# AlphacatPlus/VmambaIR

Hardware: AMD Instinct MI355X
Metric: images/sec, x4 SR 64->256 training step (fwd+bwd+Adam+EMA), full VmambaIR UNet (higher is better)
Workload: dtype bf16; 1 GPU; BASELINE.json configs[1]: x4 SR 64x64 LQ, MambaSISR6 dim48 [15,1,1,1]+15, bf16 autocast (scan arithmetic f32), batch 8 per GPU; global_batch=8, per_gpu_batch=8, parallelism=dp1, step_launch=hipGraph replay, vendor_conv_solver_search=True, vendor_conv_solver_records=bench_data/miopen, optimizer=Adam 2e-4 (0.9,0.99) + EMA 0.999, loss=L1, rccl_ranks=1, allreduce_overlapped=False, allreduce_buckets=1, allreduce_bytes=0

## Files before the change

### include/vmambair_oss.h

```cpp
#ifndef VMAMBAIR_OSS_H
#define VMAMBAIR_OSS_H

#include <stddef.h>
#include <stdint.h>

#ifdef __cplusplus
extern "C" {
#endif

#define OSS_OK 0
#define OSS_ERR_NULL (-1)
#define OSS_ERR_SHAPE (-2)
#define OSS_ERR_DSTATE (-3)
#define OSS_ERR_WORKSPACE (-4)

#define OSS_MAX_DSTATE 256

typedef enum {
    OSS_F32 = 0, OSS_F16 = 1, OSS_BF16 = 2,
    OSS_F32_BF16X3 = 3
} oss_dtype;

typedef void *oss_stream_t;

// ... 101 lines not shown
                   float *dweight, float *dbias, float *partials, int batch, int hidden, int height, int width,
                   int64_t t_batch_stride, int64_t t_channel_stride, int64_t dout_batch_stride, int64_t dout_channel_stride,
                   int64_t dt_batch_stride, int64_t dt_channel_stride, oss_stream_t stream);

int oss_dwconv3x3_flat2_ok(oss_dtype io, int height, int width);
int oss_dwconv3x3_silu_flat2_fwd(oss_dtype io, const void *x, const float *weight, const float *bias, void *x2, int batch, int channels,
                                 int height, int width, int64_t x_batch_stride, int64_t x_channel_stride, oss_stream_t stream);
int oss_dwconv3x3_silu_flat2_bwd(oss_dtype io, const void *x, const float *weight, const float *bias, const void *g2, void *dx,
                                 float *dweight, float *dbias, float *partials, int batch, int channels, int height, int width,
                                 int64_t x_batch_stride, int64_t x_channel_stride, int64_t dx_batch_stride, int64_t dx_channel_stride,
                                 oss_stream_t stream);

int oss_conv1x1_fwd(oss_dtype io, const void *x, const float *weight, const float *bias, const void *residual, void *y,
                    int batch, int cout, int cin, int pixels, int64_t x_batch_stride, int64_t x_channel_stride,
                    oss_stream_t stream);
int oss_conv1x1_dgrad(oss_dtype io, const void *dy, const float *weight, void *dx, int batch, int cout, int cin, int pixels,
                      int64_t dy_batch_stride, int64_t dy_channel_stride, oss_stream_t stream);
size_t oss_conv1x1_wgrad_partial_floats(int batch, int cout, int cin, int pixels);
int oss_conv1x1_wg(oss_dtype io, const void *x, const float *weight, const float *bias, void *y, int batch, int cout, int cin,
                   int pixels, int64_t x_batch_stride, int64_t x_channel_stride, int transposed_weight, oss_stream_t stream);
int oss_ln_conv1x1_ok(oss_dtype io, int cout, int cin, int pixels);
int oss_ln_conv1x1_fwd(oss_dtype io, const void *x, const float *ln_weight, const float *ln_bias, float eps, void *n, float *mean,
                       float *rstd, const float *weight, const float *bias, void *y, int batch, int cout, int cin, int pixels,
                       int64_t x_batch_stride, int64_t x_channel_stride, oss_stream_t stream);
int oss_conv1x1_dgrad_ln_bwd_ok(oss_dtype io, int cout, int cin, int pixels, int batch);
size_t oss_conv1x1_dgrad_ln_bwd_partial_floats(int batch, int cin, int pixels);
int oss_conv1x1_dgrad_ln_bwd(oss_dtype io, const void *dy, const float *weight, const void *x, const float *ln_weight, int ln_has_bias,
                             const float *mean, const float *rstd, const void *skip_grad, void *dx, float *dln_weight, float *dln_bias,
                             float *partials, int batch, int cout, int cin, int pixels, int64_t dy_batch_stride,
                             int64_t dy_channel_stride, oss_stream_t stream);
void oss_conv1x1_set_wg(int on, int pixels);
void oss_conv1x1_wgrad_set_tile(int mode);
void oss_conv1x1_wgrad_set_span(int mult);
int oss_conv1x1_wgrad(oss_dtype io, const void *dy, const void *x, float *dweight, float *dbias, float *partials, int batch,
                      int cout, int cin, int pixels, int64_t dy_batch_stride, int64_t dy_channel_stride,
                      int64_t x_batch_stride, int64_t x_channel_stride, oss_stream_t stream);

int oss_cross_scan2(oss_dtype in_type, oss_dtype out_type, const void *x, void *x2, int batch, int D, int height, int width,
                    int64_t x_batch_stride, int64_t x_channel_stride, oss_stream_t stream);
int oss_cross_merge2(oss_dtype io, const void *g2, void *dx, int batch, int D, int height, int width, oss_stream_t stream);
int oss_proj_fwd(oss_dtype io, const void *x2, const float *x_proj_weight, const float *dt_projs_weight, void *xdbl, void *dts,
                 int batch, int D, int C, int R, int seqlen, oss_stream_t stream);
int oss_proj_dgrad(oss_dtype io, const void *ddts, void *dxdbl, const void *du, const float *x_proj_weight,
                   const float *dt_projs_weight, void *dx2, int batch, int D, int C, int R, int seqlen, oss_stream_t stream);
size_t oss_proj_wgrad_partial_floats(int batch, int D, int C, int R, int seqlen);
void oss_proj_set_path(int force_vector_alu);
int oss_proj_rows_optional_ok(oss_dtype io, int batch, int D, int C, int R, int seqlen);
int oss_proj_wgrad(oss_dtype io, const void *x2, const void *xdbl, const void *dxdbl, const void *ddts, float *dx_proj_weight,
                   float *ddt_projs_weight, float *partials, int batch, int D, int C, int R, int seqlen, oss_stream_t stream);

typedef struct {
    int B, L, dc, Rc, Cc, reserved_;
    const float *pooled;
    const float *cin_w, *cin_b;
    const float *Wxc;
    const float *Wdtc;
    const float *dt_bias;
    const float *A_logs;
    const float *Dsc;
    const float *cout_w, *cout_b;
    const float *cn_w, *cn_b;
    float *zt;
    float *dts;
    float *hs;
    float *y;
    float *yc;
// ... 131 lines not shown
```

### vmambair_amd/csrc/oss_capi.hip

```cpp
#include <atomic>
#include <cstdlib>
#include <mutex>
#include <vector>
#include <cstring>
#include <algorithm>
#include "oss_device.h"
#include "oss_host.h"

namespace oss {

static std::atomic<int> g_force_fwd{-1}, g_force_bwd{-1};
static std::atomic<int> g_last_fwd{-1}, g_last_bwd{-1};
static std::atomic<int> g_force_fwd_seg{-1}, g_force_bwd_seg{-1};
std::atomic<int> g_last_fwd_segments{1}, g_last_bwd_segments{1}, g_last_bwd_lane_states{0};

int scan_pick_segments(long wgs, int n_chunks, int seg_req, double ovh) {
    if (seg_req == 0 || seg_req == 1 || n_chunks < 2 || wgs <= 0) return 1;
    if (seg_req > 1) return std::min(std::min(seg_req, n_chunks), kMaxSegments);
    if (wgs >= 256) return 1;
    int best = 1;
    double best_cost = (double)n_chunks;
    for (int s = 2; s <= std::min(n_chunks, 16); ++s) {
        const int cps = (n_chunks + s - 1) / s;
        if ((n_chunks + cps - 1) / cps != s) continue;
// ... 487 lines not shown
int oss_ln_conv1x1_fwd(oss_dtype io, const void *x, const float *ln_weight, const float *ln_bias, float eps, void *n, float *mean,
                       float *rstd, const float *weight, const float *bias, void *y, int batch, int cout, int cin, int pixels,
                       int64_t xsb, int64_t xsc, oss_stream_t stream) {
    if (is_f32_split(io)) return OSS_ERR_SHAPE;
    fam_count(FAM_CONV1X1, (double)batch * pixels * (esz(io) * (2.0 * cin + cout) + 8.0) + 4.0 * cin * cout);
    if (!x || !ln_weight || !n || !mean || !rstd || !weight || !y) return OSS_ERR_NULL;
    if (batch <= 0 || batch > 65535) return OSS_ERR_SHAPE;
    return ln_conv1x1_wg(io, x, ln_weight, ln_bias, eps, n, mean, rstd, weight, bias, y, batch, cout, cin, pixels, xsb, xsc,
                         reinterpret_cast<hipStream_t>(stream));
}

int oss_conv1x1_dgrad_ln_bwd_ok(oss_dtype io, int cout, int cin, int pixels, int batch) {
    if (is_f32_split(io)) return 0;
    return conv1x1_dgrad_lnbwd_ok(io, cin, cout, pixels, batch);
}
size_t oss_conv1x1_dgrad_ln_bwd_partial_floats(int batch, int cin, int pixels) {
    if (batch <= 0 || cin <= 0 || pixels <= 0) return 0;
    return conv1x1_dgrad_lnbwd_partial_floats(batch, cin, pixels);
}
int oss_conv1x1_dgrad_ln_bwd(oss_dtype io, const void *dy, const float *weight, const void *x, const float *ln_weight, int ln_has_bias,
                             const float *mean, const float *rstd, const void *skip_grad, void *dx, float *dln_weight, float *dln_bias,
                             float *partials, int batch, int cout, int cin, int pixels, int64_t gsb, int64_t gsc, oss_stream_t stream) {
    if (is_f32_split(io)) return OSS_ERR_SHAPE;
    fam_count(FAM_CONV1X1, (double)batch * pixels * (esz(io) * ((double)cout + 2.0 * cin + (skip_grad ? cin : 0)) + 8.0) + 4.0 * cin * cout);
    if (!dy || !weight || !x || !ln_weight || !mean || !rstd || !dx || !dln_weight || !partials) return OSS_ERR_NULL;
    if (batch <= 0 || batch > 65535) return OSS_ERR_SHAPE;
    return conv1x1_dgrad_lnbwd(io, dy, weight, x, ln_weight, ln_has_bias, mean, rstd, skip_grad, dx, dln_weight, dln_bias, partials, batch,
                               cin, cout, pixels, gsb, gsc, reinterpret_cast<hipStream_t>(stream));
}

void oss_conv1x1_set_wg(int on, int pixels) { conv1x1_set_wg(on); conv1x1_wg_set_pixels(pixels); }
void oss_conv1x1_wgrad_set_tile(int mode) { conv1x1_wgrad_set_tile(mode); }
void oss_conv1x1_wgrad_set_span(int mult) { conv1x1_wgrad_set_span(mult); }

int oss_proj_wgrad(oss_dtype io, const void *x2, const void *xdbl, const void *dxdbl, const void *ddts, float *dx_proj_weight,
                   float *ddt_projs_weight, float *partials, int batch, int D, int C, int R, int seqlen, oss_stream_t stream) {
    const int x3 = take_f32_split(io);
    fam_count(FAM_WGRAD, (double)batch * seqlen * esz(io) * (2.0 * D + 8.0 * C + (ddts ? 4.0 * D : 0.0)));
    if (!x2 || !xdbl || !dxdbl || !dx_proj_weight || !partials) return OSS_ERR_NULL;
    if (ddts && !ddt_projs_weight) return OSS_ERR_NULL;
    if (batch <= 0 || D <= 0 || seqlen <= 0 || R <= 0 || C <= R) return OSS_ERR_SHAPE;
    hipStream_t s = reinterpret_cast<hipStream_t>(stream);
    const int64_t L = seqlen;
    if (io == OSS_F32) {
        int e = rows_f32_wgrad(reinterpret_cast<const float *>(dxdbl), reinterpret_cast<const float *>(x2), dx_proj_weight, partials, batch,
                               4, 2, C, D, seqlen, 4 * C * L, C * L, L, 2 * D * L, D * L, L, s, nullptr, x3);
        if (e || !ddts) return e;
        float *part2 = partials + (size_t)batch * conv1x1_wgrad_slabs(seqlen) * 2 * (2 * (size_t)C) * D;
        return rows_f32_wgrad(reinterpret_cast<const float *>(ddts), reinterpret_cast<const float *>(xdbl), ddt_projs_weight, part2, batch, 4,
                              4, D, R, seqlen, 4 * D * L, D * L, L, 4 * C * L, C * L, L, s, nullptr, x3);
    }
    int e = conv1x1_wgrad(io, dxdbl, x2, dx_proj_weight, partials, batch, 2 * C, D, seqlen, 4 * C * L, L, 2 * D * L, L, s,
                           2,  C * L,  D * L,  C,  2 * C * L);
    if (e || !ddts) return e;
    float *part2 = partials + (size_t)batch * conv1x1_wgrad_slabs(seqlen) * 2 * (2 * (size_t)C) * D;
    return conv1x1_wgrad(io, ddts, xdbl, ddt_projs_weight, part2, batch, D, R, seqlen, 4 * D * L, L, 4 * C * L, L, s,
                          4,  D * L,  C * L,  D, 0);
}

int oss_cross_scan2(oss_dtype in_type, oss_dtype out_type, const void *x, void *x2, int batch, int D, int height, int width,
                    int64_t x_batch_stride, int64_t x_channel_stride, oss_stream_t stream) {
    if (is_f32_split(in_type) || is_f32_split(out_type)) return OSS_ERR_SHAPE;
    fam_count(FAM_MERGE, (double)batch * D * height * width * (esz(in_type) + 2.0 * esz(out_type)));
    if (!x || !x2) return OSS_ERR_NULL;
    if (batch <= 0 || D <= 0 || height <= 0 || width <= 0) return OSS_ERR_SHAPE;
    return cross_scan2(in_type, out_type, x, x2, batch, D, height, width, x_batch_stride, x_channel_stride,
// ... 455 lines not shown
```

### vmambair_amd/csrc/oss_conv1x1.hip

```cpp
#include <atomic>
#include <cstdlib>
#include "oss_device.h"
#include "oss_global_ptr.h"
#include "oss_host.h"
#include "oss_mfma.h"

namespace oss {

template <typename T>
__global__ void __launch_bounds__(256)
oss_conv1x1_kernel(const T *__restrict__ x, const float *__restrict__ w, const float *__restrict__ bias, T *__restrict__ y,
                   int M, int K, int P, int64_t xsb, int64_t xsk, int64_t ws_m, int64_t ws_k, const T *__restrict__ res) {
    const int lane = threadIdx.x & 63, wave = threadIdx.x >> 6;
    const int b = blockIdx.y;
    const int m0 = blockIdx.z * 32;
    const int p0 = (blockIdx.x * 4 + wave) * 32;
    if (p0 >= P) return;
    const int col = lane & 31, kg = lane >> 5;
    const int p = p0 + col;
    const bool pok = p < P;
    const T *xb = x + b * xsb + (pok ? p : 0);
    T *yb = y + (size_t)b * M * P;
    const int mrow = m0 + col;
    const bool mok = mrow < M;
// ... 519 lines not shown
#pragma unroll
        for (int ks = 0; ks < KS; ++ks) {
#pragma unroll
            for (int e = 0; e < 8; ++e) {
                const int k = kc + ks * 16 + kg * 8 + e;
                const bool kok = k < K;
                const uint32_t raw = xw[(kok ? k : K - 1) * xsw];
                const uint32_t v = (pok && kok) ? raw : 0u;
                bfa[ks][e] = (short)(v & 0xffffu);
                bfb[ks][e] = (short)(v >> 16);
            }
        }
#pragma unroll
        for (int t = 0; t < MT; ++t) {
            s16x8 af[KS];
#pragma unroll
            for (int ks = 0; ks < KS; ++ks) af[ks] = load_wfrag<T, WT, WVEC>(w, (mt0 + t) * 32 + col, M, K, kc + ks * 16 + kg * 8);
            if ((mt0 + t) * 32 < M) {
#pragma unroll
                for (int ks = 0; ks < KS; ++ks) {
                    if (kc + ks * 16 < K) {
                        acca[t] = Mfma<T>::run(af[ks], bfa[ks], acca[t]);
                        accb[t] = Mfma<T>::run(af[ks], bfb[ks], accb[t]);
                    }
                }
            }
        }
    }
#pragma unroll
    for (int t = 0; t < MT; ++t)
        pair_epilogue<T>(acca[t], accb[t], bias, res ? res + (size_t)b * M * P + (pok ? p : 0) : nullptr, yb + p, (mt0 + t) * 32, kg, M, P, pok);
}

constexpr int kWgradSlab = 512;
template <typename T>
__device__ __forceinline__ void
wgrad_body(const T *__restrict__ dy, const T *__restrict__ x, float *__restrict__ part, int M, int N, int P,
           int64_t gsb, int64_t gsm, int64_t xsb, int64_t xsn, int G, int64_t gsg, int64_t xsg, int Mh,
           int64_t gs_hi, int NB ,
           int slab, int nslabs, int by, int bz, int span ) {
    const int lane = threadIdx.x & 63, wave = threadIdx.x >> 6;
    const int b = by / G, g = by - b * G;
    const int pbeg = slab * span, pend = min(P, pbeg + span);
    const int col = lane & 31, kg = lane >> 5;
    const int mt = (M + 31) >> 5, nt = (NB + 31) >> 5;
    const T *gb = dy + b * gsb + g * gsg;
    const T *xb = x + b * xsb + g * xsg;
    const size_t pvec = (size_t)G * M * N + (NB > N ? M : 0);
    float *pb = part + (size_t)(b * nslabs + slab) * pvec;
    const short kOne = (short)from_f32<T>(1.0f).v;
    const s16x8 zero8 = {0, 0, 0, 0, 0, 0, 0, 0}, ones8 = {kOne, kOne, kOne, kOne, kOne, kOne, kOne, kOne};
    const bool aligned = (((reinterpret_cast<uintptr_t>(gb) | reinterpret_cast<uintptr_t>(xb)) & 15u) == 0) &&
                         (gsm % 8 == 0) && (xsn % 8 == 0) && (pbeg % 8 == 0) && (gs_hi % 8 == 0);
    {
        const int tile = bz * 4 + wave;
        if (tile >= mt * nt) return;
        const int m0 = (tile / nt) * 32, n0 = (tile % nt) * 32;
        const int mrow = m0 + col, nrow = n0 + col;
        const bool mok = mrow < M, nok = nrow < N, one = nrow == N && NB > N;
        const int mr = mok ? mrow : 0;
        const T *ga = gb + (mr / Mh) * gs_hi + (mr % Mh) * gsm;
        const T *xa = xb + (nok ? nrow : 0) * xsn;
        f32x16 acc;
#pragma unroll
        for (int r = 0; r < 16; ++r) acc[r] = 0.f;

        int pk = pbeg;
// ... 105 lines not shown
                    const short av = (short)ga[kc].v, bv = (short)xa[kc].v;
                    af[e] = (mok && kok) ? av : (short)0;
                    bf[e] = kok ? (nok ? bv : (one ? kOne : (short)0)) : (short)0;
                }
            }
            acc = Mfma<T>::run(af, bf, acc);
        }
#pragma unroll
        for (int r = 0; r < 16; ++r) {
            const int row = m0 + (r & 3) + 8 * (r >> 2) + 4 * kg;
            const int cn = n0 + col;
#ifdef OSS_EXP_WGRAD_NOSTORE
            if (row < M && cn < NB && acc[r] == 123456.789f) {
#else
            if (row < M && cn < NB) {
#endif
                const size_t drow = ((size_t)(row / Mh) * G + g) * Mh + row % Mh;
                if (cn < N) pb[drow * N + cn] = acc[r];
                else pb[(size_t)G * M * N + row] = acc[r];
            }
        }
    }
}

template <typename T>
__global__ void __launch_bounds__(256)
oss_conv1x1_wgrad_kernel(const T *__restrict__ dy, const T *__restrict__ x, float *__restrict__ part, int M, int N, int P,
                         int64_t gsb, int64_t gsm, int64_t xsb, int64_t xsn, int G, int64_t gsg, int64_t xsg, int Mh,
                         int64_t gs_hi, int NB) {
    wgrad_body<T>(dy, x, part, M, N, P, gsb, gsm, xsb, xsn, G, gsg, xsg, Mh, gs_hi, NB, (int)blockIdx.x, (int)gridDim.x, (int)blockIdx.y,
                  (int)blockIdx.z, kWgradSlab);
}

struct WgradDesc {
    const void *dy, *x;
    float *part;
    int64_t gsb, gsm, xsb, xsn, gsg, xsg, gs_hi;
    int M, N, P, G, Mh, NB, slabs, bgs ;
    unsigned first_block;
    int io;
    int span, reserved_;
};
template <typename T>
__global__ void __launch_bounds__(256)
oss_conv1x1_wgrad_grouped_kernel(const WgradDesc *__restrict__ descs, const uint16_t *__restrict__ block_problem) {
    const WgradDesc d = descs[block_problem[blockIdx.x]];
    const unsigned local = blockIdx.x - d.first_block;
    const int slab = (int)(local % (unsigned)d.slabs);
    const unsigned r = local / (unsigned)d.slabs;
    const int by = (int)(r % (unsigned)d.bgs), bz = (int)(r / (unsigned)d.bgs);
    const WgradDesc *dt = descs + block_problem[blockIdx.x];
    wgrad_body<T>(table_ptr<const T>(&dt->dy), table_ptr<const T>(&dt->x), table_ptr<float>(&dt->part), d.M, d.N, d.P, d.gsb, d.gsm, d.xsb,
                  d.xsn, d.G, d.gsg, d.xsg, d.Mh, d.gs_hi, d.NB, slab, d.slabs, by, bz, d.span);
}

__global__ void __launch_bounds__(256)
oss_conv1x1_wgrad_finish(const float *__restrict__ part, float *__restrict__ dw, float *__restrict__ db, int nslab, size_t pvec,
                         size_t nw) {
    __shared__ float red[4][64];
    const int colx = threadIdx.x & 63, slice = threadIdx.x >> 6;
    const size_t i = (size_t)blockIdx.x * 64 + colx;
    float s = 0.f;
    if (i < pvec) {
        const float *pp = part + i;
        int k = slice;
        float s0 = 0.f, s1 = 0.f, s2 = 0.f, s3 = 0.f;
        for (; k + 12 < nslab; k += 16) {
            s0 += pp[(size_t)k * pvec];
            s1 += pp[(size_t)(k + 4) * pvec];
            s2 += pp[(size_t)(k + 8) * pvec];
            s3 += pp[(size_t)(k + 12) * pvec];
        }
        for (; k < nslab; k += 4) s0 += pp[(size_t)k * pvec];
        s = (s0 + s1) + (s2 + s3);
    }
    red[slice][colx] = s;
    __syncthreads();
    if (slice == 0 && i < pvec) {
        const float t = (red[0][colx] + red[1][colx]) + (red[2][colx] + red[3][colx]);
        if (i < nw) dw[i] = t;
        else db[i - nw] = t;
    }
}

static long conv1x1_target_waves() {
    static const long v = [] {
        const char *e = getenv("VMAMBAIR_CONV1X1_WAVES");
        const long t = e ? atol(e) : 0;
// ... 269 lines not shown
#undef OSS_WG
}

int conv1x1_wgrad_slabs(int P) { return (P + kWgradSlab - 1) / kWgradSlab; }

static std::atomic<int> g_wgrad_span{-1};
static int wgrad_span_mult() {
    int m = g_wgrad_span.load();
    if (m < 0) {
        const char *e = std::getenv("VMAMBAIR_WGRAD_SPAN");
        m = e ? std::atoi(e) : 4;
        m = m < 1 ? 1 : (m > 64 ? 64 : m);
        g_wgrad_span.store(m);
    }
    return m;
}
void conv1x1_wgrad_set_span(int mult) { g_wgrad_span.store(mult < 1 ? 1 : (mult > 64 ? 64 : mult)); }

int conv1x1_wgrad(oss_dtype io, const void *dy, const void *x, float *dw, float *part, int B, int M, int N, int P,
                  int64_t gsb, int64_t gsm, int64_t xsb, int64_t xsn, hipStream_t s, int G, int64_t gsg, int64_t xsg, int Mh,
                  int64_t gs_hi, float *db, int f32_split) {
    const int NB = N + (db ? 1 : 0);
    if (G < 1 || (size_t)B * G > 65535) return OSS_ERR_SHAPE;
    if (io == OSS_F32) {
        if (G != 1 || (Mh > 0 && Mh != M)) return OSS_ERR_SHAPE;
        return rows_f32_wgrad(reinterpret_cast<const float *>(dy), reinterpret_cast<const float *>(x), dw, part, B, 1, 1, M, N, P, gsb, 0,
                              gsm, xsb, 0, xsn, s, db, f32_split);
    }
    if (Mh <= 0 || Mh > M) Mh = M;
    int slabs = conv1x1_wgrad_slabs(P);
    const int tiles = ((M + 31) / 32) * ((NB + 31) / 32);
    dim3 grid(slabs, B * G, (tiles + 3) / 4);
    const int tmode = wgrad_tile_mode();
    if (defer_wgrad() && !tmode && (io == OSS_BF16 || io == OSS_F16) && (size_t)slabs * B * G * ((tiles + 3) / 4) < (1u << 24)) {
        if (!defer_finish()) return OSS_ERR_WORKSPACE;
        WgradDesc d;
        d.span = kWgradSlab * wgrad_span_mult(); d.reserved_ = 0;
        slabs = (P + d.span - 1) / d.span;
        d.dy = dy; d.x = x; d.part = part;
        d.gsb = gsb; d.gsm = gsm; d.xsb = xsb; d.xsn = xsn; d.gsg = gsg; d.xsg = xsg; d.gs_hi = gs_hi;
        d.M = M; d.N = N; d.P = P; d.G = G; d.Mh = Mh; d.NB = NB; d.slabs = slabs; d.bgs = B * G;
        d.first_block = 0; d.io = (int)io;
        defer_wgrad_push(&d, sizeof(d), (unsigned)(slabs * B * G * ((tiles + 3) / 4)));
    } else
    if (tmode && (io == OSS_BF16 || io == OSS_F16)) {
        if (io == OSS_BF16)
            wgrad_tiles_launch<bf16_t>(tmode, reinterpret_cast<const bf16_t *>(dy), reinterpret_cast<const bf16_t *>(x), part, B, M, N, P,
                                       gsb, gsm, xsb, xsn, G, gsg, xsg, Mh, gs_hi, NB, slabs, s);
        else
            wgrad_tiles_launch<f16_t>(tmode, reinterpret_cast<const f16_t *>(dy), reinterpret_cast<const f16_t *>(x), part, B, M, N, P,
                                      gsb, gsm, xsb, xsn, G, gsg, xsg, Mh, gs_hi, NB, slabs, s);
    } else
    switch (io) {
        case OSS_BF16:
            hipLaunchKernelGGL(oss_conv1x1_wgrad_kernel<bf16_t>, grid, dim3(256), 0, s, reinterpret_cast<const bf16_t *>(dy),
                               reinterpret_cast<const bf16_t *>(x), part, M, N, P, gsb, gsm, xsb, xsn, G, gsg, xsg, Mh, gs_hi, NB);
            break;
        case OSS_F16:
            hipLaunchKernelGGL(oss_conv1x1_wgrad_kernel<f16_t>, grid, dim3(256), 0, s, reinterpret_cast<const f16_t *>(dy),
                               reinterpret_cast<const f16_t *>(x), part, M, N, P, gsb, gsm, xsb, xsn, G, gsg, xsg, Mh, gs_hi, NB);
            break;
        default: return OSS_ERR_SHAPE;
    }
    if (db && G != 1) return OSS_ERR_SHAPE;
    const size_t nw = (size_t)G * M * N, pvec = nw + (db ? M : 0);
    if (defer_finish())
        defer_sum(part, slabs * B, pvec, pvec, dw, nw, db);
    else
        hipLaunchKernelGGL(oss_conv1x1_wgrad_finish, dim3((unsigned)((pvec + 63) / 64)), dim3(256), 0, s, part, dw, db, slabs * B,
                           pvec, nw);
    return (int)hipGetLastError();
}

size_t wgrad_desc_bytes() { return sizeof(WgradDesc); }
int wgrad_grouped_launch(int io, const void *d_descs, const void *d_map, unsigned total_blocks, hipStream_t s) {
    if (total_blocks == 0) return 0;
    if (io == OSS_BF16)
        hipLaunchKernelGGL(oss_conv1x1_wgrad_grouped_kernel<bf16_t>, dim3(total_blocks), dim3(256), 0, s,
                           reinterpret_cast<const WgradDesc *>(d_descs), reinterpret_cast<const uint16_t *>(d_map));
    else if (io == OSS_F16)
        hipLaunchKernelGGL(oss_conv1x1_wgrad_grouped_kernel<f16_t>, dim3(total_blocks), dim3(256), 0, s,
                           reinterpret_cast<const WgradDesc *>(d_descs), reinterpret_cast<const uint16_t *>(d_map));
    else
        return OSS_ERR_SHAPE;
    return (int)hipGetLastError();
}
void wgrad_desc_set_first_block(void *desc, unsigned first) { reinterpret_cast<WgradDesc *>(desc)->first_block = first; }
int wgrad_desc_io(const void *desc) { return reinterpret_cast<const WgradDesc *>(desc)->io; }

}
```

### vmambair_amd/csrc/oss_host.h

```cpp
#pragma once
#include <hip/hip_runtime.h>
#include "../../include/vmambair_oss.h"

#include <atomic>
#include <initializer_list>

namespace oss {
struct bf16_t;
struct f16_t;

constexpr size_t kMaxLdsBytes = 160 * 1024;
struct LdsGate {
    std::atomic<size_t> enabled[16] = {};
    int ensure(const void *kern, size_t bytes) {
        if (bytes <= 48 * 1024) return 0;
        if (bytes > kMaxLdsBytes) return OSS_ERR_SHAPE;
        int dev = 0;
        (void)hipGetDevice(&dev);
        std::atomic<size_t> &slot = enabled[dev & 15];
        if (bytes <= slot.load(std::memory_order_acquire)) return 0;
        const hipError_t e = hipFuncSetAttribute(kern, hipFuncAttributeMaxDynamicSharedMemorySize, (int)bytes);
        if (e != hipSuccess) return (int)e;
        size_t cur = slot.load(std::memory_order_relaxed);
        while (cur < bytes && !slot.compare_exchange_weak(cur, bytes, std::memory_order_release)) {}
// ... 71 lines not shown
int conv3x3_thin_fwd(oss_dtype io, const void *x, const float *w, const float *bias, void *y, int B, int Cin, int Cout, int H, int W,
                     int64_t xsb, int64_t xsc, int64_t ysb, int64_t ysc, hipStream_t s);
int conv3x3_thin_dgrad(oss_dtype io, const void *dy, const float *w, void *dx, int B, int Cin, int Cout, int H, int W, int64_t gsb,
                       int64_t gsc, int64_t dsb, int64_t dsc, hipStream_t s);
size_t conv3x3_thin_wgrad_partial_floats(int B, int Cin, int Cout);
int conv3x3_thin_wgrad(oss_dtype io, const void *x, const void *dy, float *dw, float *db, float *part, int B, int Cin, int Cout, int H,
                       int W, int64_t xsb, int64_t xsc, int64_t gsb, int64_t gsc, hipStream_t s);
int ln_nchw_fwd(oss_dtype xt, oss_dtype yt, const void *x, const float *w, const float *bias, const void *gate, void *y,
                float *mean, float *rstd, int B, int C, int P, int64_t xsb, int64_t xsc, int64_t gsb, int64_t gsc, float eps,
                hipStream_t s, float *pool_part = nullptr);
int ln_nchw_fwd_pool_tiles(int C, int P, int64_t xsb, int64_t xsc, int64_t gsb, int64_t gsc);
size_t ln_nchw_bwd_partial_floats(int B, int C, int P);
int ln_nchw_bwd(oss_dtype xt, oss_dtype yt, const void *x, const float *w, const float *bias, const void *gate,
                const void *dy, const float *mean, const float *rstd, void *dx, void *dgate, float *dw, float *db,
                float *part, int B, int C, int P, int64_t xsb, int64_t xsc, int64_t gsb, int64_t gsc, hipStream_t s,
                const void *res = nullptr, int64_t dgsb = 0, const float *dy_mul = nullptr, const float *dy_add = nullptr,
                float add_scale = 1.f);
int merge4(oss_dtype io, const void *out, float *y, int B, int D, int H, int W, hipStream_t s);
int ln_conv1x1_wg(oss_dtype io, const void *x, const float *ln_w, const float *ln_b, float eps, void *n, float *mean, float *rstd,
                  const float *w, const float *bias, void *y, int B, int M, int K, int P, int64_t xsb, int64_t xsk, hipStream_t s);
size_t conv1x1_dgrad_lnbwd_partial_floats(int B, int M, int P);
int conv1x1_dgrad_lnbwd_ok(oss_dtype io, int M, int K, int P, int B);
int conv1x1_dgrad_lnbwd(oss_dtype io, const void *dy, const float *w, const void *x, const float *ln_w, int with_bias, const float *mean,
                        const float *rstd, const void *skip, void *dx, float *dlw, float *dlb, float *part, int B, int M, int K, int P,
                        int64_t xsb, int64_t xsk, hipStream_t s);
void conv1x1_set_wg(int on);
void conv1x1_wg_set_pixels(int pt);
int conv1x1_wg_ok(oss_dtype io, int M, int K, int P, int64_t xsb, int64_t xsk, const void *x, const void *y, const float *w,
                  const void *res = nullptr);
int conv1x1_wg(oss_dtype io, const void *x, const float *w, const float *bias, void *y, int B, int M, int K, int P, int64_t xsb,
               int64_t xsk, int wt, hipStream_t s, const void *res = nullptr);
int conv1x1(oss_dtype io, const void *x, const float *w, const float *bias, void *y, int B, int M, int K, int P, int64_t xsb,
            int64_t xsk, int64_t ws_m, int64_t ws_k, hipStream_t s, const void *res = nullptr, int f32_split = 0);
int conv1x1_wgrad_slabs(int P);
void conv1x1_wgrad_set_tile(int mode);
void conv1x1_wgrad_set_span(int mult);
int conv1x1_wgrad(oss_dtype io, const void *dy, const void *x, float *dw, float *part, int B, int M, int N, int P,
                  int64_t gsb, int64_t gsm, int64_t xsb, int64_t xsn, hipStream_t s, int G = 1, int64_t gsg = 0, int64_t xsg = 0,
                  int Mh = 0, int64_t gs_hi = 0, float *db = nullptr, int f32_split = 0);
int proj_fwd(oss_dtype io, const void *x2, const float *Wx, const float *Wdt, void *xdbl, void *dts, int B, int D, int C, int R,
             int L, hipStream_t s, int f32_split = 0);
int proj_dgrad(oss_dtype io, const void *ddts, void *dxdbl, const void *du, const float *Wx, const float *Wdt, void *dx2, int B,
               int D, int C, int R, int L, hipStream_t s, int f32_split = 0);
void proj_force_valu(int on);
bool proj_mfma_ok(oss_dtype io, int B, int D, int C, int R, int L);
int cross_scan2(oss_dtype it, oss_dtype ot, const void *x, void *x2, int B, int D, int H, int W, int64_t xsb, int64_t xsc,
                hipStream_t s);
int cross_merge2(oss_dtype io, const void *g2, void *dx, int B, int D, int H, int W, hipStream_t s);
size_t chan_grad_floats(int L, int dc, int Rc, int Cc);
size_t chan_bwd_scratch_floats(int B, int L, int dc, int Rc, int Cc);
int chan_fwd(const oss_chan_params &p, hipStream_t s);
int chan_bwd(const oss_chan_params &p, const float *gc, float *dpool, float *gsum, float *scratch, hipStream_t s);
int rowsum(oss_dtype io, const void *a, const void *bmul, float *out, int B, int C, int P, int64_t asb, int64_t asc, int64_t bsb,
           int64_t bsc, float alpha, hipStream_t s);
int row_affine(oss_dtype io, const void *x, const float *mul, const float *add, void *y, int B, int C, int P, int64_t xsb,
               int64_t xsc, float alpha, hipStream_t s);
int gelu_gate_fwd(oss_dtype io, const void *h, void *out, int B, size_t n, int64_t hsb, hipStream_t s);
int gelu_gate_bwd(oss_dtype io, const void *h, const void *dout, void *dh, int B, size_t n, int64_t hsb, int64_t gsb, hipStream_t s);
bool defer_wgrad();
void defer_wgrad_push(const void *desc, size_t bytes, unsigned blocks);
size_t wgrad_desc_bytes();
int wgrad_grouped_launch(int io, const void *d_descs, const void *d_map, unsigned total_blocks, hipStream_t s);
void wgrad_desc_set_first_block(void *desc, unsigned first);
int wgrad_desc_io(const void *desc);
bool defer_finish();
void defer_sum(const float *src, int K, size_t stride, size_t V, float *dst0, size_t n0, float *dst1);
int sum_partials_multi(const oss_sum_chunk *chunks, int n_chunks, hipStream_t s);
int adam_ema_step(const oss_adam_chunk *chunks, int n_chunks, float *state, float lr, float beta1, float beta2, float eps,
                  float ema_decay, hipStream_t s, float weight_decay = 0.f, const float *grad_scale = nullptr);
int image_metrics_ok(oss_dtype io, int C, int H, int W, int crop, int flags);
size_t image_metrics_partial_doubles(int B, int C, int H, int W, int crop);
int image_metrics(oss_dtype io, const void *a, const void *b, double *out, double *part, int B, int C, int H, int W, int64_t asb,
                  int64_t asc, int64_t ars, int64_t bsb, int64_t bsc, int64_t brs, int crop, int flags, hipStream_t s);
int scan_fwd_pick_variant(int batch, int dim, int seqlen, int dstate, int n_groups, int elem_bytes);
}
```

Baseline: 245.3 images/s.

## Register-block grouped conv1x1 wgrad with LDS-staged buffer loads and multi-tile waves

Moves the grouped (deferred) conv1x1 weight-gradient kernel into its own file and rewrites its body so each wave computes a block of up to 3x1 or 2x2 32x32 MFMA tiles, reusing loaded dy/x fragments across tiles. Full slabs are streamed with raw buffer loads into a per-wave LDS staging area and double-buffered fragment reads. The block shape defaults to a heuristic that can be overridden by an environment variable or setter. The cost is more registers and 72KB of LDS per workgroup, which limits occupancy, plus a new 29-bit offset limit that sends large problems back to the old path.

```diff
diff --git a/include/vmambair_oss.h b/include/vmambair_oss.h
--- a/include/vmambair_oss.h
+++ b/include/vmambair_oss.h
@@ -157,6 +157,7 @@
 void oss_conv1x1_set_wg(int on, int pixels);
 void oss_conv1x1_wgrad_set_tile(int mode);
 void oss_conv1x1_wgrad_set_span(int mult);
+void oss_conv1x1_wgrad_set_block(int mode);
 int oss_conv1x1_wgrad(oss_dtype io, const void *dy, const void *x, float *dweight, float *dbias, float *partials, int batch,
                       int cout, int cin, int pixels, int64_t dy_batch_stride, int64_t dy_channel_stride,
                       int64_t x_batch_stride, int64_t x_channel_stride, oss_stream_t stream);
diff --git a/vmambair_amd/csrc/oss_capi.hip b/vmambair_amd/csrc/oss_capi.hip
--- a/vmambair_amd/csrc/oss_capi.hip
+++ b/vmambair_amd/csrc/oss_capi.hip
@@ -543,6 +543,7 @@
 void oss_conv1x1_set_wg(int on, int pixels) { conv1x1_set_wg(on); conv1x1_wg_set_pixels(pixels); }
 void oss_conv1x1_wgrad_set_tile(int mode) { conv1x1_wgrad_set_tile(mode); }
 void oss_conv1x1_wgrad_set_span(int mult) { conv1x1_wgrad_set_span(mult); }
+void oss_conv1x1_wgrad_set_block(int mode) { conv1x1_wgrad_set_block(mode); }
 
 int oss_proj_wgrad(oss_dtype io, const void *x2, const void *xdbl, const void *dxdbl, const void *ddts, float *dx_proj_weight,
                    float *ddt_projs_weight, float *partials, int batch, int D, int C, int R, int seqlen, oss_stream_t stream) {
diff --git a/vmambair_amd/csrc/oss_conv1x1.hip b/vmambair_amd/csrc/oss_conv1x1.hip
--- a/vmambair_amd/csrc/oss_conv1x1.hip
+++ b/vmambair_amd/csrc/oss_conv1x1.hip
@@ -575,7 +575,6 @@
         pair_epilogue<T>(acca[t], accb[t], bias, res ? res + (size_t)b * M * P + (pok ? p : 0) : nullptr, yb + p, (mt0 + t) * 32, kg, M, P, pok);
 }
 
-constexpr int kWgradSlab = 512;
 template <typename T>
 __device__ __forceinline__ void
 wgrad_body(const T *__restrict__ dy, const T *__restrict__ x, float *__restrict__ part, int M, int N, int P,
@@ -747,28 +746,6 @@
                   (int)blockIdx.z, kWgradSlab);
 }
 
-struct WgradDesc {
-    const void *dy, *x;
-    float *part;
-    int64_t gsb, gsm, xsb, xsn, gsg, xsg, gs_hi;
-    int M, N, P, G, Mh, NB, slabs, bgs ;
-    unsigned first_block;
-    int io;
-    int span, reserved_;
-};
-template <typename T>
-__global__ void __launch_bounds__(256)
-oss_conv1x1_wgrad_grouped_kernel(const WgradDesc *__restrict__ descs, const uint16_t *__restrict__ block_problem) {
-    const WgradDesc d = descs[block_problem[blockIdx.x]];
-    const unsigned local = blockIdx.x - d.first_block;
-    const int slab = (int)(local % (unsigned)d.slabs);
-    const unsigned r = local / (unsigned)d.slabs;
-    const int by = (int)(r % (unsigned)d.bgs), bz = (int)(r / (unsigned)d.bgs);
-    const WgradDesc *dt = descs + block_problem[blockIdx.x];
-    wgrad_body<T>(table_ptr<const T>(&dt->dy), table_ptr<const T>(&dt->x), table_ptr<float>(&dt->part), d.M, d.N, d.P, d.gsb, d.gsm, d.xsb,
-                  d.xsn, d.G, d.gsg, d.xsg, d.Mh, d.gs_hi, d.NB, slab, d.slabs, by, bz, d.span);
-}
-
 __global__ void __launch_bounds__(256)
 oss_conv1x1_wgrad_finish(const float *__restrict__ part, float *__restrict__ dw, float *__restrict__ db, int nslab, size_t pvec,
                          size_t nw) {
@@ -1104,16 +1081,13 @@
     const int tiles = ((M + 31) / 32) * ((NB + 31) / 32);
     dim3 grid(slabs, B * G, (tiles + 3) / 4);
     const int tmode = wgrad_tile_mode();
+    bool recorded = false;
     if (defer_wgrad() && !tmode && (io == OSS_BF16 || io == OSS_F16) && (size_t)slabs * B * G * ((tiles + 3) / 4) < (1u << 24)) {
         if (!defer_finish()) return OSS_ERR_WORKSPACE;
-        WgradDesc d;
-        d.span = kWgradSlab * wgrad_span_mult(); d.reserved_ = 0;
-        slabs = (P + d.span - 1) / d.span;
-        d.dy = dy; d.x = x; d.part = part;
-        d.gsb = gsb; d.gsm = gsm; d.xsb = xsb; d.xsn = xsn; d.gsg = gsg; d.xsg = xsg; d.gs_hi = gs_hi;
-        d.M = M; d.N = N; d.P = P; d.G = G; d.Mh = Mh; d.NB = NB; d.slabs = slabs; d.bgs = B * G;
-        d.first_block = 0; d.io = (int)io;
-        defer_wgrad_push(&d, sizeof(d), (unsigned)(slabs * B * G * ((tiles + 3) / 4)));
+        const int rs = wgrad_record(io, dy, x, part, B, M, N, P, gsb, gsm, xsb, xsn, G, gsg, xsg, Mh, gs_hi, NB, wgrad_span_mult());
+        if (rs > 0) { slabs = rs; recorded = true; }
+    }
+    if (recorded) {
     } else
     if (tmode && (io == OSS_BF16 || io == OSS_F16)) {
         if (io == OSS_BF16)
@@ -1144,20 +1118,4 @@
     return (int)hipGetLastError();
 }
 
-size_t wgrad_desc_bytes() { return sizeof(WgradDesc); }
-int wgrad_grouped_launch(int io, const void *d_descs, const void *d_map, unsigned total_blocks, hipStream_t s) {
-    if (total_blocks == 0) return 0;
-    if (io == OSS_BF16)
-        hipLaunchKernelGGL(oss_conv1x1_wgrad_grouped_kernel<bf16_t>, dim3(total_blocks), dim3(256), 0, s,
-                           reinterpret_cast<const WgradDesc *>(d_descs), reinterpret_cast<const uint16_t *>(d_map));
-    else if (io == OSS_F16)
-        hipLaunchKernelGGL(oss_conv1x1_wgrad_grouped_kernel<f16_t>, dim3(total_blocks), dim3(256), 0, s,
-                           reinterpret_cast<const WgradDesc *>(d_descs), reinterpret_cast<const uint16_t *>(d_map));
-    else
-        return OSS_ERR_SHAPE;
-    return (int)hipGetLastError();
-}
-void wgrad_desc_set_first_block(void *desc, unsigned first) { reinterpret_cast<WgradDesc *>(desc)->first_block = first; }
-int wgrad_desc_io(const void *desc) { return reinterpret_cast<const WgradDesc *>(desc)->io; }
-
-}
+}
diff --git a/vmambair_amd/csrc/oss_conv1x1_wgrad_grouped.hip b/vmambair_amd/csrc/oss_conv1x1_wgrad_grouped.hip
--- /dev/null
+++ b/vmambair_amd/csrc/oss_conv1x1_wgrad_grouped.hip
@@ -0,0 +1,320 @@
+#include <algorithm>
+#include <atomic>
+#include <cstdlib>
+#include "oss_device.h"
+#include "oss_global_ptr.h"
+#include "oss_host.h"
+#include "oss_mfma.h"
+
+namespace oss {
+
+struct WgradDesc {
+    const void *dy, *x;
+    float *part;
+    int64_t gsb, gsm, xsb, xsn, gsg, xsg, gs_hi;
+    int M, N, P, G, Mh, NB, slabs, bgs ;
+    unsigned first_block;
+    int io;
+    int span;
+    int block;
+};
+
+template <typename T>
+__device__ __forceinline__ __amdgpu_buffer_rsrc_t wave_buffer(const T *p, unsigned bytes) {
+    const uint64_t v = reinterpret_cast<uint64_t>(p);
+    const uint64_t u = ((uint64_t)(uint32_t)__builtin_amdgcn_readfirstlane((int)(uint32_t)(v >> 32)) << 32) |
+                       (uint32_t)__builtin_amdgcn_readfirstlane((int)(uint32_t)v);
+    return __builtin_amdgcn_make_buffer_rsrc(reinterpret_cast<void *>(u), 0, (int)bytes, 0x00020000);
+}
+constexpr int kWgradBlockTiles = 4;
+template <typename T, int TM, int TN>
+__device__ __forceinline__ void
+wgrad_block_body(const T *__restrict__ dy, const T *__restrict__ x, float *__restrict__ part, int M, int N, int P, int64_t gsb,
+                 int64_t gsm, int64_t xsb, int64_t xsn, int G, int64_t gsg, int64_t xsg, int Mh, int64_t gs_hi, int NB, int slab,
+                 int nslabs, int by, int m0, int n0 , int span,
+                 T *__restrict__ st ) {
+    static_assert(TM + TN <= kWgradBlockTiles, "the wave's LDS region holds kWgradBlockTiles * 32 rows");
+    const int lane = threadIdx.x & 63;
+    const int b = by / G, g = by - b * G;
+    const int pbeg = slab * span, pend = min(P, pbeg + span);
+    const int col = lane & 31, kg = lane >> 5;
+    const T *gb = dy + b * gsb + g * gsg;
+    const T *xb = x + b * xsb + g * xsg;
+    const size_t pvec = (size_t)G * M * N + (NB > N ? M : 0);
+    float *pb = part + (size_t)(b * nslabs + slab) * pvec;
+    const short kOne = (short)from_f32<T>(1.0f).v;
+    const s16x8 zero8 = {0, 0, 0, 0, 0, 0, 0, 0}, ones8 = {kOne, kOne, kOne, kOne, kOne, kOne, kOne, kOne};
+    const bool aligned = (((reinterpret_cast<uintptr_t>(gb) | reinterpret_cast<uintptr_t>(xb)) & 15u) == 0) &&
+                         (gsm % 8 == 0) && (xsn % 8 == 0) && (pbeg % 8 == 0) && (gs_hi % 8 == 0);
+    const int ml = m0 + 32 * (TM - 1), nl = n0 + 32 * (TN - 1);
+    const bool mokl = ml + col < M, nokl = nl + col < N, onel = nl + col == N && NB > N;
+    f32x16 acc[TM][TN];
+#pragma unroll
+    for (int i = 0; i < TM; ++i)
+#pragma unroll
+        for (int j = 0; j < TN; ++j)
+#pragma unroll
+            for (int r = 0; r < 16; ++r) acc[i][j][r] = 0.f;
+
+    int pk = pbeg;
+    if (aligned && pend - pk >= kWgradSlab) {
+        constexpr int PIECES = kWgradSlab / 64, RS = 72, GA = 4 * TM, NG = 4 * (TM + TN);
+        constexpr int WIN = NG <= 8 ? 4 : 1;
+        const int r8 = lane >> 3, q = lane & 7;
+        constexpr unsigned kOutside = 0x80000000u;
+        unsigned vo[NG];
+#pragma unroll
+        for (int j = 0; j < NG; ++j) {
+            if (j < GA) {
+                const int row = m0 + 8 * j + r8;
+                const int64_t off = (row / Mh) * gs_hi + (row % Mh) * gsm + q * 8;
+                vo[j] = (j < GA - 4 || row < M) ? (unsigned)(off * (int64_t)sizeof(T)) : kOutside;
+            } else {
+                const int row = n0 + 8 * (j - GA) + r8;
+                vo[j] = (j < NG - 4 || row < N) ? (unsigned)((row * xsn + q * 8) * (int64_t)sizeof(T)) : kOutside;
+            }
+        }
+        T *sw = st + r8 * RS + q * 8;
+        const T *sr = st + col * RS + kg * 8;
+        for (; pend - pk >= kWgradSlab; pk += kWgradSlab) {
+            const __amdgpu_buffer_rsrc_t rg = wave_buffer(gb + pk, kOutside), rx = wave_buffer(xb + pk, kOutside);
+            u32x4 w[WIN][NG];
+#pragma unroll
+            for (int pc = 0; pc < WIN; ++pc)
+#pragma unroll
+                for (int j = 0; j < NG; ++j)
+                    w[pc][j] = __builtin_bit_cast(u32x4, __builtin_amdgcn_raw_buffer_load_b128(j < GA ? rg : rx, vo[j] + pc * 128, 0, 0));
+#pragma unroll
+            for (int pc = 0; pc < PIECES; ++pc) {
+#pragma unroll
+                for (int j = 0; j < NG; ++j) *reinterpret_cast<u32x4 *>(sw + 8 * j * RS) = w[pc % WIN][j];
+                if (pc + WIN < PIECES) {
+#pragma unroll
+                    for (int j = 0; j < NG; ++j)
+                        w[pc % WIN][j] = __builtin_bit_cast(u32x4, __builtin_amdgcn_raw_buffer_load_b128(j < GA ? rg : rx,
+                                                                                                         vo[j] + (pc + WIN) * 128, 0, 0));
+                }
+                __builtin_amdgcn_wave_barrier();
+                u32x4 fa[2][TM], fb[2][TN];
+#pragma unroll
+                for (int i = 0; i < TM; ++i) fa[0][i] = *reinterpret_cast<const u32x4 *>(sr + 32 * i * RS);
+#pragma unroll
+                for (int j = 0; j < TN; ++j) fb[0][j] = *reinterpret_cast<const u32x4 *>(sr + 32 * (TM + j) * RS);
+#pragma unroll
+                for (int u = 0; u < 4; ++u) {
+                    if (u < 3) {
+#pragma unroll
+                        for (int i = 0; i < TM; ++i) fa[(u + 1) & 1][i] = *reinterpret_cast<const u32x4 *>(sr + 32 * i * RS + (u + 1) * 16);
+#pragma unroll
+                        for (int j = 0; j < TN; ++j)
+                            fb[(u + 1) & 1][j] = *reinterpret_cast<const u32x4 *>(sr + 32 * (TM + j) * RS + (u + 1) * 16);
+                    }
+                    s16x8 af[TM], bf[TN];
+#pragma unroll
+                    for (int i = 0; i < TM; ++i) af[i] = (i < TM - 1 || mokl) ? __builtin_bit_cast(s16x8, fa[u & 1][i]) : zero8;
+#pragma unroll
+                    for (int j = 0; j < TN; ++j)
+                        bf[j] = (j < TN - 1 || nokl) ? __builtin_bit_cast(s16x8, fb[u & 1][j]) : (onel ? ones8 : zero8);
+#pragma unroll
+                    for (int i = 0; i < TM; ++i)
+#pragma unroll
+                        for (int j = 0; j < TN; ++j) acc[i][j] = Mfma<T>::run(af[i], bf[j], acc[i][j]);
+                }
+                __builtin_amdgcn_wave_barrier();
+            }
+        }
+    }
+    if (pk < pend) {
+        bool mok[TM], nok[TN], one[TN];
+        const T *ga[TM], *xa[TN];
+#pragma unroll
+        for (int i = 0; i < TM; ++i) {
+            mok[i] = i < TM - 1 || mokl;
+            const int mr = mok[i] ? m0 + 32 * i + col : 0;
+            ga[i] = gb + (mr / Mh) * gs_hi + (mr % Mh) * gsm;
+        }
+#pragma unroll
+        for (int j = 0; j < TN; ++j) {
+            nok[j] = j < TN - 1 || nokl;
+            one[j] = j == TN - 1 && onel;
+            xa[j] = xb + (nok[j] ? n0 + 32 * j + col : 0) * xsn;
+        }
+        if (aligned) {
+            for (; pk + 64 <= pend; pk += 64) {
+                u32x4 qa[TM][4], qb[TN][4];
+#pragma unroll
+                for (int u = 0; u < 4; ++u) {
+#pragma unroll
+                    for (int i = 0; i < TM; ++i) qa[i][u] = *reinterpret_cast<const u32x4 *>(ga[i] + pk + u * 16 + kg * 8);
+#pragma unroll
+                    for (int j = 0; j < TN; ++j) qb[j][u] = *reinterpret_cast<const u32x4 *>(xa[j] + pk + u * 16 + kg * 8);
+                }
+#pragma unroll
+                for (int u = 0; u < 4; ++u)
+#pragma unroll
+                    for (int i = 0; i < TM; ++i)
+#pragma unroll
+                        for (int j = 0; j < TN; ++j) {
+                            const s16x8 af = mok[i] ? __builtin_bit_cast(s16x8, qa[i][u]) : zero8;
+                            const s16x8 bf = nok[j] ? __builtin_bit_cast(s16x8, qb[j][u]) : (one[j] ? ones8 : zero8);
+                            acc[i][j] = Mfma<T>::run(af, bf, acc[i][j]);
+                        }
+            }
+        }
+        for (; pk < pend; pk += 16) {
+            const int k0 = pk + kg * 8;
+            const bool vec = aligned && k0 + 8 <= pend;
+            s16x8 af[TM], bf[TN];
+#pragma unroll
+            for (int i = 0; i < TM; ++i) {
+                if (vec) {
+                    const u32x4 qa = *reinterpret_cast<const u32x4 *>(ga[i] + k0);
+                    af[i] = mok[i] ? __builtin_bit_cast(s16x8, qa) : zero8;
+                } else {
+#pragma unroll
+                    for (int e = 0; e < 8; ++e) {
+                        const bool kok = (k0 + e) < pend;
+                        const short av = (short)ga[i][kok ? k0 + e : pend - 1].v;
+                        af[i][e] = (mok[i] && kok) ? av : (short)0;
+                    }
+                }
+            }
+#pragma unroll
+            for (int j = 0; j < TN; ++j) {
+                if (vec) {
+                    const u32x4 qb = *reinterpret_cast<const u32x4 *>(xa[j] + k0);
+                    bf[j] = nok[j] ? __builtin_bit_cast(s16x8, qb) : (one[j] ? ones8 : zero8);
+                } else {
+#pragma unroll
+                    for (int e = 0; e < 8; ++e) {
+                        const bool kok = (k0 + e) < pend;
+                        const short bv = (short)xa[j][kok ? k0 + e : pend - 1].v;
+                        bf[j][e] = kok ? (nok[j] ? bv : (one[j] ? kOne : (short)0)) : (short)0;
+                    }
+                }
+            }
+#pragma unroll
+            for (int i = 0; i < TM; ++i)
+#pragma unroll
+                for (int j = 0; j < TN; ++j) acc[i][j] = Mfma<T>::run(af[i], bf[j], acc[i][j]);
+        }
+    }
+#pragma unroll
+    for (int i = 0; i < TM; ++i)
+#pragma unroll
+        for (int j = 0; j < TN; ++j) {
+#pragma unroll
+            for (int r = 0; r < 16; ++r) {
+                const int row = m0 + 32 * i + (r & 3) + 8 * (r >> 2) + 4 * kg;
+                const int cn = n0 + 32 * j + col;
+                if (row < M && cn < NB) {
+                    const size_t drow = ((size_t)(row / Mh) * G + g) * Mh + row % Mh;
+                    if (cn < N) pb[drow * N + cn] = acc[i][j][r];
+                    else pb[(size_t)G * M * N + row] = acc[i][j][r];
+                }
+            }
+        }
+}
+
+template <typename T>
+__global__ void __launch_bounds__(256, 2)
+oss_conv1x1_wgrad_grouped_kernel(const WgradDesc *__restrict__ descs, const uint16_t *__restrict__ block_problem) {
+    __shared__ __attribute__((aligned(16))) T stage[4][kWgradBlockTiles * 32 * 72];
+    const WgradDesc d = descs[block_problem[blockIdx.x]];
+    const unsigned local = blockIdx.x - d.first_block;
+    const int wave = __builtin_amdgcn_readfirstlane((int)(threadIdx.x >> 6));
+    const WgradDesc *dt = descs + block_problem[blockIdx.x];
+    const int tm = d.block ? d.block / 10 : 1, tn = d.block ? d.block % 10 : 1;
+    const int mt = (d.M + 31) >> 5, nt = (d.NB + 31) >> 5;
+    const int nbk = (nt + tn - 1) / tn;
+    const unsigned nblk = (unsigned)(((mt + tm - 1) / tm) * nbk);
+    unsigned slab, by, blk;
+    if (d.block == 0) {
+        slab = local % (unsigned)d.slabs;
+        const unsigned r = local / (unsigned)d.slabs;
+        by = r % (unsigned)d.bgs;
+        blk = r / (unsigned)d.bgs * 4 + (unsigned)wave;
+        if (blk >= nblk) return;
+    } else {
+        const unsigned item = local * 4 + (unsigned)wave;
+        blk = item % nblk;
+        const unsigned r = item / nblk;
+        slab = r % (unsigned)d.slabs;
+        by = r / (unsigned)d.slabs;
+        if (by >= (unsigned)d.bgs) return;
+    }
+    const int mi = (int)(blk / (unsigned)nbk) * tm, ni = (int)(blk % (unsigned)nbk) * tn;
+    const int am = min(tm, mt - mi), an = min(tn, nt - ni);
+#define OSS_WGB(TM_, TN_)                                                                                                              \
+    wgrad_block_body<T, TM_, TN_>(table_ptr<const T>(&dt->dy), table_ptr<const T>(&dt->x), table_ptr<float>(&dt->part), d.M, d.N, d.P,  \
+                                  d.gsb, d.gsm, d.xsb, d.xsn, d.G, d.gsg, d.xsg, d.Mh, d.gs_hi, d.NB, (int)slab, d.slabs, (int)by,      \
+                                  32 * mi, 32 * ni, d.span, stage[wave])
+    switch (am * 10 + an) {
+        case 11: OSS_WGB(1, 1); break;
+        case 21: OSS_WGB(2, 1); break;
+        case 31: OSS_WGB(3, 1); break;
+        case 12: OSS_WGB(1, 2); break;
+        case 22: OSS_WGB(2, 2); break;
+        default: break;
+    }
+#undef OSS_WGB
+}
+
+static int wgrad_block_valid(int m) { return (m == 0 || m == 11 || m == 21 || m == 31 || m == 12 || m == 22) ? m : -1; }
+static std::atomic<int> g_wgrad_block{-2};
+static int wgrad_block_mode() {
+    int m = g_wgrad_block.load();
+    if (m < -1) {
+        const char *e = std::getenv("VMAMBAIR_WGRAD_BLOCK");
+        m = (e && *e) ? wgrad_block_valid(std::atoi(e)) : -1;
+        g_wgrad_block.store(m);
+    }
+    return m;
+}
+void conv1x1_wgrad_set_block(int mode) { g_wgrad_block.store(wgrad_block_valid(mode)); }
+static int wgrad_block_shape(int mt, int nt) {
+    const int mode = wgrad_block_mode();
+    if (mode >= 0) return mode;
+    if (mt % 3 == 0 || mt < 3) return std::min(mt, 3) * 10 + 1;
+    return 20 + (nt < 2 ? 1 : 2);
+}
+
+int wgrad_record(oss_dtype io, const void *dy, const void *x, float *part, int B, int M, int N, int P, int64_t gsb, int64_t gsm,
+                 int64_t xsb, int64_t xsn, int G, int64_t gsg, int64_t xsg, int Mh, int64_t gs_hi, int NB, int span_mult) {
+    const int64_t hi = (int64_t)((M - 1) / Mh) * gs_hi + (int64_t)(Mh - 1) * gsm, xhi = (int64_t)(N - 1) * xsn;
+    if (gs_hi < 0 || gsm < 0 || xsn < 0 || hi + P + 8 * (gs_hi + gsm) >= (1ll << 29) || xhi + P + 8 * xsn >= (1ll << 29)) return -1;
+    WgradDesc d;
+    d.span = kWgradSlab * span_mult;
+    const int slabs = (P + d.span - 1) / d.span;
+    const int mt = (M + 31) / 32, nt = (NB + 31) / 32;
+    d.block = wgrad_block_shape(mt, nt);
+    d.dy = dy; d.x = x; d.part = part;
+    d.gsb = gsb; d.gsm = gsm; d.xsb = xsb; d.xsn = xsn; d.gsg = gsg; d.xsg = xsg; d.gs_hi = gs_hi;
+    d.M = M; d.N = N; d.P = P; d.G = G; d.Mh = Mh; d.NB = NB; d.slabs = slabs; d.bgs = B * G;
+    d.first_block = 0; d.io = (int)io;
+    size_t wgs = (size_t)slabs * B * G * ((mt * nt + 3) / 4);
+    if (d.block) {
+        const int tm = d.block / 10, tn = d.block % 10;
+        wgs = ((size_t)slabs * B * G * ((mt + tm - 1) / tm) * ((nt + tn - 1) / tn) + 3) / 4;
+    }
+    defer_wgrad_push(&d, sizeof(d), (unsigned)wgs);
+    return slabs;
+}
+
+size_t wgrad_desc_bytes() { return sizeof(WgradDesc); }
+int wgrad_grouped_launch(int io, const void *d_descs, const void *d_map, unsigned total_blocks, hipStream_t s) {
+    if (total_blocks == 0) return 0;
+    if (io == OSS_BF16)
+        hipLaunchKernelGGL(oss_conv1x1_wgrad_grouped_kernel<bf16_t>, dim3(total_blocks), dim3(256), 0, s,
+                           reinterpret_cast<const WgradDesc *>(d_descs), reinterpret_cast<const uint16_t *>(d_map));
+    else if (io == OSS_F16)
+        hipLaunchKernelGGL(oss_conv1x1_wgrad_grouped_kernel<f16_t>, dim3(total_blocks), dim3(256), 0, s,
+                           reinterpret_cast<const WgradDesc *>(d_descs), reinterpret_cast<const uint16_t *>(d_map));
+    else
+        return OSS_ERR_SHAPE;
+    return (int)hipGetLastError();
+}
+void wgrad_desc_set_first_block(void *desc, unsigned first) { reinterpret_cast<WgradDesc *>(desc)->first_block = first; }
+int wgrad_desc_io(const void *desc) { return reinterpret_cast<const WgradDesc *>(desc)->io; }
+
+}
diff --git a/vmambair_amd/csrc/oss_host.h b/vmambair_amd/csrc/oss_host.h
--- a/vmambair_amd/csrc/oss_host.h
+++ b/vmambair_amd/csrc/oss_host.h
@@ -127,9 +127,11 @@
                int64_t xsk, int wt, hipStream_t s, const void *res = nullptr);
 int conv1x1(oss_dtype io, const void *x, const float *w, const float *bias, void *y, int B, int M, int K, int P, int64_t xsb,
             int64_t xsk, int64_t ws_m, int64_t ws_k, hipStream_t s, const void *res = nullptr, int f32_split = 0);
+constexpr int kWgradSlab = 512;
 int conv1x1_wgrad_slabs(int P);
 void conv1x1_wgrad_set_tile(int mode);
 void conv1x1_wgrad_set_span(int mult);
+void conv1x1_wgrad_set_block(int mode);
 int conv1x1_wgrad(oss_dtype io, const void *dy, const void *x, float *dw, float *part, int B, int M, int N, int P,
                   int64_t gsb, int64_t gsm, int64_t xsb, int64_t xsn, hipStream_t s, int G = 1, int64_t gsg = 0, int64_t xsg = 0,
                   int Mh = 0, int64_t gs_hi = 0, float *db = nullptr, int f32_split = 0);
@@ -155,6 +157,8 @@
 bool defer_wgrad();
 void defer_wgrad_push(const void *desc, size_t bytes, unsigned blocks);
 size_t wgrad_desc_bytes();
+int wgrad_record(oss_dtype io, const void *dy, const void *x, float *part, int B, int M, int N, int P, int64_t gsb, int64_t gsm,
+                 int64_t xsb, int64_t xsn, int G, int64_t gsg, int64_t xsg, int Mh, int64_t gs_hi, int NB, int span_mult);
 int wgrad_grouped_launch(int io, const void *d_descs, const void *d_map, unsigned total_blocks, hipStream_t s);
 void wgrad_desc_set_first_block(void *desc, unsigned first);
 int wgrad_desc_io(const void *desc);
```

Result: no change. 246.4 images/s (median of 6 runs) (+0.5%).
